# rensonnetg/microstructure_fingerprinting

Hardware: AMD Instinct MI355X
Metric: voxels/sec, 2-fascicle exhaustive NNLS, 782-atom x 200-measurement dictionary (higher is better)
Workload: dtype f64 (pairs ranked on split-f16 MFMA, short list re-evaluated in f64); 1 GPU; C2: 100000 voxels/GPU, 2 fascicles, 782 atoms x 200 measurements; voxels_per_gpu=100000, global_voxels=100000, atoms=782, measurements=200, ranks_in_group=1

## Files before the change

### microstructure_fingerprinting_amd/_lib.py

```python
import ctypes as C
import os

import numpy as np

_HERE = os.path.dirname(os.path.abspath(__file__))
LIB_PATH = os.path.join(_HERE, "libmfx.so")

MFX_OK, MFX_ERR_ARG, MFX_ERR_G_RANGE, MFX_ERR_NO_DEVICE, MFX_ERR_HIP, MFX_ERR_UNSUPPORTED, MFX_ERR_DIR_NORM = range(7)

_lib = None

EXPORTS = [
    "mfx_last_error", "mfx_device_count", "mfx_abi_version",
    "mfx_tables_create", "mfx_tables_destroy", "mfx_tables_num_atoms",
    "mfx_plan_create_multishell", "mfx_plan_create_explicit", "mfx_plan_destroy", "mfx_plan_status",
    "mfx_rotate", "mfx_rotate_dev", "mfx_rotate_cols", "mfx_rotate_cols_dev", "mfx_fit_batch", "mfx_fit_batch_rows", "mfx_fit_batch_volume", "mfx_volume_rows", "mfx_thread_release", "mfx_fit_batch_dev",
    "mfx_solve_exhaustive", "mfx_monte_carlo_average", "mfx_monte_carlo_average_dev", "mfx_cleanup_2fascicles", "mfx_cleanup_2fascicles_dev", "mfx_last_kernel_ms", "mfx_set_profiling", "mfx_debug_set_stamps", "mfx_debug_last_fallback_count", "mfx_debug_last_guard_count", "mfx_debug_last_counter", "mfx_debug_set_k2_screen", "mfx_debug_set_k2_wide", "mfx_debug_set_k2x_screen", "mfx_debug_set_k2_maxc", "mfx_debug_set_k2x_maxc", "mfx_debug_set_k2s_cap", "mfx_debug_set_k2s_images", "mfx_debug_set_k3_cap", "mfx_debug_set_force_generic", "mfx_debug_set_k3_screen",
]

MCF_EXPORTS = ["mfx_mcf_abi_version", "mfx_mcf_pgse", "mfx_mcf_dde"]

ROT2D_EXPORTS = ["mfx_rot2d_abi_version", "mfx_rot2d_create", "mfx_rot2d_destroy", "mfx_rot2d_rotate",
                 "mfx_rot2d_rotate_dev", "mfx_rot2d_rotate_cols", "mfx_rot2d_rotate_cols_dev"]

# ... 6 lines not shown
PREDICT_EXPORTS = ["mfx_predict_abi_version", "mfx_predict_dev", "mfx_predict", "mfx_sos_noise_dev", "mfx_sos_noise"]

PROFILE_EXPORTS = ["mfx_profile_abi_version", "mfx_profile_cut", "mfx_profile_max_atoms", "mfx_profile_dev", "mfx_profile",
                   "mfx_pair_objectives_dev", "mfx_pair_objectives"]

POST_EXPORTS = ["mfx_post_abi_version", "mfx_post_max_atoms", "mfx_post_dev", "mfx_post"]

WSOFT_EXPORTS = ["mfx_wsoft_abi_version", "mfx_wsoft_max_atoms", "mfx_wpost_dev", "mfx_wpost", "mfx_wprofile_dev", "mfx_wprofile",
                 "mfx_wpair_objectives_dev", "mfx_wpair_objectives"]

SOFT2D_EXPORTS = ["mfx_soft2d_abi_version", "mfx_soft2d_max_atoms", "mfx_post2d_dev", "mfx_post2d", "mfx_profile2d_dev",
                  "mfx_profile2d"]

W2D_EXPORTS = ["mfx_w2d_abi_version", "mfx_w2d_max_atoms", "mfx_wfit2d_batch_dev", "mfx_wfit2d_batch", "mfx_wpost2d_dev",
               "mfx_wpost2d", "mfx_wprofile2d_dev", "mfx_wprofile2d", "mfx_w2d_debug_set_force_explicit"]


class MfxError(RuntimeError):
    pass


def lib():
    global _lib
    if _lib is not None:
        return _lib
    if not os.path.exists(LIB_PATH):
        raise MfxError("HIP extension %s not found: run `python -c 'import __graft_entry__ as g; g.build()'` "
                       "(or `make -C microstructure_fingerprinting_amd/csrc`). There is no CPU fallback." % LIB_PATH)
    L = C.CDLL(LIB_PATH)
    dp = C.POINTER(C.c_double)
# ... 46 lines not shown
    L.mfx_debug_set_k2_wide.restype = None
    L.mfx_debug_set_k2x_screen.argtypes = [C.c_int]
    L.mfx_debug_set_k2x_screen.restype = None
    L.mfx_debug_set_k2_maxc.argtypes = [C.c_int]
    L.mfx_debug_set_k2_maxc.restype = None
    L.mfx_debug_set_k2s_cap.argtypes = [C.c_int]
    L.mfx_debug_set_k2s_cap.restype = None
    L.mfx_debug_set_k3_cap.argtypes = [C.c_int]
    L.mfx_debug_set_k3_cap.restype = None
    L.mfx_debug_set_force_generic.argtypes = [C.c_int]
    L.mfx_debug_set_force_generic.restype = None
    L.mfx_debug_set_k3_screen.argtypes = [C.c_int]
    L.mfx_debug_set_k3_screen.restype = None
    L.mfx_debug_set_k2s_images.argtypes = [C.c_int]
    L.mfx_debug_set_k2s_images.restype = None
    L.mfx_mcf_abi_version.restype = C.c_int
    for fn in ("mfx_mcf_pgse", "mfx_mcf_dde"):
        getattr(L, fn).argtypes = [dp, dp, C.c_int, dp, C.c_int64, dp, dp, C.c_int64, dp, C.c_double, dp]
        getattr(L, fn).restype = C.c_int
    L.mfx_rot2d_abi_version.restype = C.c_int
    L.mfx_rot2d_create.argtypes = [dp, C.c_int, ip, ip, C.c_int, ip, dp, ip, ip, ip, dp, C.c_int, ip, dp, dp, C.c_int,
                                   C.c_int, C.c_double, C.c_double, C.c_int, C.POINTER(vp)]
    L.mfx_rot2d_destroy.argtypes = [vp]
    L.mfx_rot2d_destroy.restype = None
    L.mfx_rot2d_rotate.argtypes = [vp, dp, C.c_int64, dp, ip]
    L.mfx_rot2d_rotate_dev.argtypes = [vp, vp, C.c_int64, vp, vp, vp]
    L.mfx_rot2d_rotate_cols.argtypes = [vp, dp, ip, C.c_int64, dp, ip]
    L.mfx_rot2d_rotate_cols_dev.argtypes = [vp, vp, vp, C.c_int64, vp, vp, vp]
    L.mfx_fit2d_abi_version.restype = C.c_int
    L.mfx_fit2d_max_atoms.argtypes = [vp, C.c_int]
# ... 88 lines not shown
```

### microstructure_fingerprinting_amd/csrc/fit_k2.hip

```cpp
#pragma once
#include <type_traits>

#include "mfx_device.h"
#include "nnls_small.h"

typedef double d4 __attribute__((ext_vector_type(4)));

#define MFX_WG 512
#define MFX_MAXC 256
#define MFX_S_CAP 2048
#define MFX_DET_REL 1e-8
#define MFX_A12_REL 4e-14

struct FitK2Args {
  TablesDev T;
  PlanDev P;
  const double* Y;
  const double* peaks;
  int peaks_ld;
  const int* vox_list;
  const int* list_count;
  double* params;
  int num_params;
  int maxfasc;
  int csf_on, ear_on;
  unsigned long long* stamps;
  int* fb_count;
  int* fb_list;
  int maxc;
  int scap;
  const double* xc;
  struct Cand* xl_cand;
  int* xl_cnt;
  double* xl_mrg;
  int xl_cap;
  int vox_base;
  int* audit;
};

#ifdef MFX_STAMPS
#define MFX_STAMP(i) do { if (a.stamps && tid == 0) a.stamps[(size_t)blockIdx.x * 16 + (i)] = __builtin_amdgcn_s_memtime(); } while (0)
#else
#define MFX_STAMP(i) do { } while (0)
#endif

struct Cand {
  double score;
  int i, j;
};

__device__ __forceinline__ double wave_max(double v) {
#pragma unroll
// ... 560 lines not shown
```

### microstructure_fingerprinting_amd/csrc/k2s_launch.h

```cpp
#pragma once
#include "mfx_host.h"
#include "fit_k2s.hip"

template <int KS, bool BR, int NB>
static int launch_k2s_t(const FitK2Args& a, int nvox, hipStream_t st) {
  MfxThread& T = mfx_thread();
  const size_t lds = mfx_k2s_lds_bytes(KS, a.T.N, BR, NB);
  auto kern = mfx_fit_k2s_kernel<KS, BR, NB>;
  HIPCHK(hipFuncSetAttribute((const void*)kern, hipFuncAttributeMaxDynamicSharedMemorySize, (int)lds));
  StreamMem fbm(st);
  HIPCHK(fbm.alloc(sizeof(int) * ((size_t)nvox + 8)));
  int* fb = fbm.as<int>();
  HIPCHK(hipMemsetAsync(fb, 0, 8 * sizeof(int), st));
  if (int rc = mfx_prof_begin(st)) return rc;
  FitK2Args aa = a;
  aa.stamps = T.stamps;
  aa.fb_count = fb;
  aa.fb_list = fb + 8;
  aa.audit = fb + 2;
  aa.scap = T.k2s_cap ? T.k2s_cap : MFX_S_CAP;
  hipLaunchKernelGGL(kern, dim3(nvox), dim3(512), lds, st, aa);
  HIPCHK(hipGetLastError());
  if (int rc = mfx_prof_end(st)) return rc;
  FitK2Args ab = a;
  ab.vox_list = fb + 8;
  ab.list_count = fb;
  if (int rc = mfx_launch_k2_f64(ab, nvox, st, false)) return rc;
  if (int rc = mfx_fb_accumulate(fb, 2, st)) return rc;
  return mfx_fb_accumulate_audit(fb + 2, st);
}

#define MFX_K2S_TU(KS_, NAME_)                                                            \
  int NAME_(const FitK2Args& a, int nvox, hipStream_t st, bool br, int NB) {              \
    if (NB == 3) return br ? launch_k2s_t<KS_, true, 3>(a, nvox, st) : launch_k2s_t<KS_, false, 3>(a, nvox, st); \
    return br ? launch_k2s_t<KS_, true, 2>(a, nvox, st) : launch_k2s_t<KS_, false, 2>(a, nvox, st);              \
// ... 2 lines not shown
```

### microstructure_fingerprinting_amd/csrc/k2s_shared.h

```cpp
#pragma once

template <int KS, int NB, bool BR, bool XC, int PQF>
struct K2sLds {
  static constexpr int MP = KS * 16;
  double* smem;
  _Float16* sBh;
  _Float16* sBl;
  double* s_y;
  double* s_t0;
  double* s_red;
  Cand* s_cand;
  unsigned long long* s_thr;
  int* s_r0;
  int* s_cnt;
  float* s_t0f;
  float* s_Zf;
  float* s_cs;
  float* s_yf;
  float* s_pq;
  double* s_t1;
  double* s_tG;
  double* s_dG;
  int* s_r1;
  int* s_rs;
// ... 7 lines not shown
    s_t0 = s_y + MP;
    s_red = s_t0 + 2 * MP;
    s_cand = (Cand*)(s_red + 32);
    s_thr = (unsigned long long*)(s_cand + MFX_S_CAP);
    s_r0 = (int*)(s_thr + 2);
    s_cnt = s_r0 + 2 * MP;
    s_t0f = (float*)(s_cnt + 4);
    s_Zf = s_t0f + 2 * MP;
    s_cs = s_Zf + 2 * NP;
    s_yf = s_cs + 2 * NP;
    s_pq = s_yf + MP;
    s_t1 = (double*)(s_pq + PQF);
    s_tG = s_t1 + (BR ? 2 * MP : 0);
    s_dG = s_tG + (BR ? MP : 0);
    s_r1 = (int*)(s_dG + (BR ? MP : 0));
    s_rs = BR ? s_r1 + 2 * MP : s_r0;
    s_evl4 = s_r1 + (BR ? 4 * MP : 0);
    s_xf = (float*)(s_evl4 + (KS < 8 ? MFX_S_CAP : 0));
    s_uf = s_xf + (XC ? MP : 0);
  }
};
#define K2S_UNPACK(L) \
  [[maybe_unused]] _Float16* const sBh = (L).sBh; \
  [[maybe_unused]] _Float16* const sBl = (L).sBl; \
  [[maybe_unused]] double* const s_y = (L).s_y; \
  [[maybe_unused]] double* const s_t0 = (L).s_t0; \
  [[maybe_unused]] double* const s_red = (L).s_red; \
  [[maybe_unused]] Cand* const s_cand = (L).s_cand; \
  [[maybe_unused]] unsigned long long* const s_thr = (L).s_thr; \
  [[maybe_unused]] int* const s_r0 = (L).s_r0; \
  [[maybe_unused]] int* const s_cnt = (L).s_cnt; \
  [[maybe_unused]] float* const s_t0f = (L).s_t0f; \
  [[maybe_unused]] float* const s_Zf = (L).s_Zf; \
  [[maybe_unused]] float* const s_cs = (L).s_cs; \
  [[maybe_unused]] float* const s_yf = (L).s_yf; \
  [[maybe_unused]] float* const s_pq = (L).s_pq; \
  [[maybe_unused]] double* const s_t1 = (L).s_t1; \
  [[maybe_unused]] double* const s_tG = (L).s_tG; \
  [[maybe_unused]] double* const s_dG = (L).s_dG; \
  [[maybe_unused]] int* const s_r1 = (L).s_r1; \
  [[maybe_unused]] int* const s_rs = (L).s_rs; \
  [[maybe_unused]] int* const s_evl4 = (L).s_evl4; \
  [[maybe_unused]] float* const s_xf = (L).s_xf; \
  [[maybe_unused]] float* const s_uf = (L).s_uf;

struct K2sVoxel {
  double y_sq;
  double yx;
  double ramp;
  double dc_eff;
  double mrg;
  double etol;
};

__device__ __forceinline__ unsigned k2s_audit_hash(int vox) {
  unsigned h = (unsigned)vox * 2654435761u;
  h ^= h >> 15; h *= 2246822519u; h ^= h >> 13; h *= 3266489917u; h ^= h >> 16;
  return h;
}
__device__ __forceinline__ int k2s_audit_key(unsigned h, int ntiles_reg, int ntiles) {
// ... 9 lines not shown
    atomicMax(&L.s_thr[1], mfx_nonneg_bits(fmin(old, 1e300)));
  }
  L.s_cand[idx].score = S;
  L.s_cand[idx].i = i;
  L.s_cand[idx].j = j;
}

template <int KS, int NB, bool BR, bool XC, int PQF, int WG>
__device__ __forceinline__ K2sVoxel k2s_prologue(const FitK2Args& a, const K2sLds<KS, NB, BR, XC, PQF>& L, const int vox, const int tid) {
  constexpr int MP = KS * 16, NW = WG / 64;
  const int lane = tid & 63, wave = tid >> 6;
  const int M = a.P.M, N = a.T.N, ldn = a.T.ldn;
  const int NP = (N + 31) & ~31;
  [[maybe_unused]] double* const smem = L.smem;
  K2S_UNPACK(L);

  MFX_STAMP(0);
  const double* __restrict__ yv = a.Y + (size_t)vox * M;
  const double* __restrict__ pk = a.peaks + (size_t)vox * a.peaks_ld;
  for (int m = tid; m < MP; m += WG) { const double v = (m < M) ? yv[m] : 0.0; s_y[m] = v; s_yf[m] = (float)v; }
  for (int idx = tid; idx < 2 * MP; idx += WG) {
    const int k = idx / MP, m = idx - k * MP;
    RowDesc rd;
    rd.r0 = a.T.P; rd.t0 = 0.0; rd.r1 = -1; rd.t1 = 0.0;
    if (m < M) rd = mfx_row_desc(a.T, a.P, m, pk[3 * k], pk[3 * k + 1], pk[3 * k + 2]);
    s_r0[idx] = rd.r0 * ldn;
    s_t0[idx] = rd.t0;
    if constexpr (!BR) {
      s_t0f[idx] = (float)rd.t0;
    } else {
      s_r1[idx] = rd.r1 < 0 ? -1 : rd.r1 * ldn;
      s_t1[idx] = rd.t1;
      if (k == 0) { s_tG[m] = (m < M) ? a.P.tG[m] : 0.0; s_dG[m] = (m < M) ? a.P.dG[m] : 1.0; }
      int rs = a.T.P;
      double ts = 0.0;
      if (m < M) {
        const int sg = a.P.s_scr[m], st = a.P.offs[2 * sg], cn = a.P.offs[2 * sg + 1];
        const double u = mfx_absdot(a.P.g + 3 * m, pk[3 * k], pk[3 * k + 1], pk[3 * k + 2]);
        int j = mfx_searchsorted_left(a.P.xs + st, cn, u);
        j = j < 1 ? 1 : (j > cn - 1 ? cn - 1 : j);
        rs = st + j - 1;
        ts = u - a.P.xs[rs];
      }
      s_rs[idx] = rs * ldn;
      s_t0f[idx] = (float)ts;
    }
  }
  if (tid == 0) { s_cnt[0] = 0; s_cnt[1] = 0; s_thr[0] = 0ull; s_thr[1] = 0ull; ((float*)(s_red + 30))[0] = __int_as_float(0x7fc00000); }
  if constexpr (XC) {
    for (int m = tid; m < MP; m += WG) s_xf[m] = (m < M) ? (float)a.xc[m] : 0.0f;
    if (tid < 2) ((unsigned long long*)s_red)[24 + tid] = 0ull;
  }
  if (tid < 2) mfx_check_dir(a.P, pk + 3 * tid, vox);
  __syncthreads();

  const float2* __restrict__ tab32 = a.P.tab32s;
  auto tab32x2_at = [&](int ro, int n) -> f32x4 { return *(const f32x4*)((const char*)tab32 + ((unsigned)(ro + n) << 3)); };

  MFX_STAMP(1);
  double y_sq_v = 0.0;
  for (int m = 0; m < M; ++m) y_sq_v += s_y[m] * s_y[m];
  const double y_sq = mfx_readlane_f64(y_sq_v, 0);
  double rsh_v = 1.0, yx_v = 0.0;
  if constexpr (XC) {
    double h = 0.0, xy = 0.0;
    for (int m = 0; m < M; ++m) { const double xv = (double)s_xf[m]; h = fma(xv, xv, h); xy = fma(xv, (double)s_yf[m], xy); }
    rsh_v = h > 0.0 ? 1.0 / sqrt(h) : 0.0;
    yx_v = xy * rsh_v;
  }
  const double rsh = mfx_readlane_f64(rsh_v, 0), yx = mfx_readlane_f64(yx_v, 0);
  const double y_sq_p = XC ? fmax(y_sq - yx * yx, 0.0) : y_sq;
  double my_s[2] = {0.0, 0.0};
  int my_n[2] = {0, 0};
  {
    const int VH = ((N + 1) / 2 + 63) & ~63;
    const int npass = (VH + WG - 1) / WG;
#pragma unroll 1
    for (int kd = XC ? 0 : 1; kd < 2; ++kd) {
    double ms_cur = 0.0, rm2_cur = 1.0;
    int mn_cur = 0;
    for (int p0 = 0; p0 < npass; p0 += 2) {
      int kq[2], nq[2];
      bool wact[2];
      double a2[2][2], ay[2][2], au[2][2];
#pragma unroll
      for (int q = 0; q < 2; ++q) {
        const int v = tid + WG * (p0 + q);
        kq[q] = kd;
        nq[q] = 2 * v;
        wact[q] = __any((p0 + q < npass) && (nq[q] < N));
        a2[q][0] = a2[q][1] = ay[q][0] = ay[q][1] = 0.0;
        au[q][0] = au[q][1] = 0.0;
      }
      int ncl[2];
#pragma unroll
      for (int q = 0; q < 2; ++q) ncl[q] = min(nq[q], ldn - 2);
      f32x4 dbuf[2][2][4];
      auto issue = [&](int m4, auto stc) {
        constexpr int st = decltype(stc)::value;
#pragma unroll
        for (int q = 0; q < 2; ++q) {
          if (wact[q]) {
            const i32x4 r = *(const i32x4*)(s_rs + kq[q] * MP + m4);
#pragma unroll
            for (int e = 0; e < 4; ++e) dbuf[st][q][e] = tab32x2_at(r[e], ncl[q]);
          }
        }
      };
      auto accumulate = [&](int m4, auto stc) {
        constexpr int st = decltype(stc)::value;
        const f32x4 yv = *(const f32x4*)(s_yf + m4);
        f32x4 xv = {0.0f, 0.0f, 0.0f, 0.0f};
        if constexpr (XC) xv = *(const f32x4*)(s_xf + m4);
#pragma unroll
        for (int q = 0; q < 2; ++q) {
          if (wact[q]) {
            const f32x4 t = *(const f32x4*)(s_t0f + kq[q] * MP + m4);
#pragma unroll
            for (int e = 0; e < 4; ++e) {
              const f32x4 d = dbuf[st][q][e];
              const double d0 = (double)fmaf(d[1], t[e], d[0]), d1 = (double)fmaf(d[3], t[e], d[2]);
              const double ye = (double)yv[e];
              a2[q][0] = fma(d0, d0, a2[q][0]);
              ay[q][0] = fma(ye, d0, ay[q][0]);
              a2[q][1] = fma(d1, d1, a2[q][1]);
              ay[q][1] = fma(ye, d1, ay[q][1]);
              if constexpr (XC) {
                const double xe = (double)xv[e];
                au[q][0] = fma(xe, d0, au[q][0]);
                au[q][1] = fma(xe, d1, au[q][1]);
              }
            }
          }
        }
      };
      issue(0, std::integral_constant<int, 0>{});
      for (int m4 = 0; m4 < MP; m4 += 8) {
        issue(m4 + 4, std::integral_constant<int, 1>{});
        accumulate(m4, std::integral_constant<int, 0>{});
        if (m4 + 8 < MP) issue(m4 + 8, std::integral_constant<int, 0>{});
        accumulate(m4 + 4, std::integral_constant<int, 1>{});
      }
#pragma unroll
      for (int q = 0; q < 2; ++q) {
#pragma unroll
        for (int u = 0; u < 2; ++u) {
          const int k = kq[q], n = nq[q] + u;
          if (p0 + q < npass && n < NP) {
            const bool act = n < N;
            if constexpr (!XC) {
              const double inv = (act && a2[q][u] > 0.0) ? 1.0 / sqrt(a2[q][u]) : 0.0;
              const double z = ay[q][u] * inv;
              s_Zf[k * NP + n] = act ? (float)z : -1e30f;
              s_cs[NP + n] = (act && inv > 0.0) ? (float)sqrt(a2[q][u]) : 0.0f;
              const double s = z > 0.0 ? z * z : 0.0;
              if (act && s > ms_cur) { ms_cur = s; mn_cur = n; }
// ... 469 lines not shown
```

### microstructure_fingerprinting_amd/csrc/k2w_launch.h

```cpp
#pragma once
#include "mfx_host.h"
#include "fit_k2w.hip"

template <int KS, int TL, bool BR, int NB>
static int launch_k2w_t(const FitK2Args& a, int nvox, hipStream_t st) {
  MfxThread& T = mfx_thread();
  const size_t lds = mfx_k2w_lds_bytes(KS, a.T.N, BR, NB, TL);
  if (lds > 160 * 1024) return mfx_fail(MFX_ERR_UNSUPPORTED, "wide K=2 kernel needs %zu B of LDS (> 160 KiB): N=%d too large", lds, a.T.N);
  auto kern = mfx_fit_k2w_kernel<KS, TL, BR, NB>;
  HIPCHK(hipFuncSetAttribute((const void*)kern, hipFuncAttributeMaxDynamicSharedMemorySize, (int)lds));
  StreamMem fbm(st);
  HIPCHK(fbm.alloc(sizeof(int) * ((size_t)nvox + 8)));
  int* fb = fbm.as<int>();
  HIPCHK(hipMemsetAsync(fb, 0, 8 * sizeof(int), st));
  if (int rc = mfx_prof_begin(st)) return rc;
  FitK2Args aa = a;
  aa.stamps = T.stamps;
  aa.fb_count = fb;
  aa.fb_list = fb + 8;
  aa.audit = fb + 2;
  aa.scap = T.k2s_cap ? T.k2s_cap : MFX_S_CAP;
  hipLaunchKernelGGL(kern, dim3(nvox), dim3(256), lds, st, aa);
  HIPCHK(hipGetLastError());
  if (int rc = mfx_prof_end(st)) return rc;
  FitK2Args ab = a;
  ab.vox_list = fb + 8;
  ab.list_count = fb;
  if (int rc = mfx_launch_k2_f64(ab, nvox, st, false)) return rc;
  if (int rc = mfx_fb_accumulate(fb, 2, st)) return rc;
  return mfx_fb_accumulate_audit(fb + 2, st);
}

#define MFX_K2W_TU(KS_, TL_, NB_, NAME_)                                                    \
  int NAME_(const FitK2Args& a, int nvox, hipStream_t st, bool br) {                        \
    return br ? launch_k2w_t<KS_, TL_, true, NB_>(a, nvox, st) : launch_k2w_t<KS_, TL_, false, NB_>(a, nvox, st); \
  }
// ... 1 lines not shown
```

### microstructure_fingerprinting_amd/csrc/mfx_api.hip

```cpp
#include "mfx_host.h"

#include <algorithm>
#include <chrono>
#include <cmath>
#include <cstdarg>
#include <cstdio>
#include <cstdlib>
#include <cstring>
#include <memory>
#include <string>
#include <vector>

#include "fit_small.hip"
#include "extras.hip"
#include "rotate.hip"
#include "solve_generic.hip"
#include "solve_k3.hip"
#include "fit_k3.hip"
#include "mc_average.hip"
#include "cleanup.hip"
#include "mfx_device.h"

MfxThread& mfx_thread() {
  static thread_local MfxThread t;
// ... 98 lines not shown
  HIPCHK(hipEventRecord(T.ev0, st));
  return MFX_OK;
}
int mfx_prof_end(hipStream_t st) {
  MfxThread& T = mfx_thread();
  if (!T.profiling) return MFX_OK;
  HIPCHK(hipEventRecord(T.ev1, st));
  T.ev_launches = 1;
  T.ev_valid = true;
  return MFX_OK;
}
__global__ void mfx_fb_add_kernel(const int* __restrict__ cnt, int n, int* __restrict__ tot) {
  if (threadIdx.x < n) atomicAdd(&tot[threadIdx.x], cnt[threadIdx.x]);
}
__global__ void mfx_fb_audit_kernel(const int* __restrict__ cnt, int* __restrict__ tot) {
  if (threadIdx.x == 0) { atomicAdd(&tot[0], cnt[0]); atomicMax(&tot[1], cnt[1]); atomicAdd(&tot[2], cnt[2]); }
}
static int fb_setup() {
  MfxThread& T = mfx_thread();
  int dev = 0;
  HIPCHK(hipGetDevice(&dev));
  if (T.fb_dev && T.fb_device == dev) return MFX_OK;
  if (T.fb_dev) { (void)hipFree(T.fb_dev); T.fb_dev = nullptr; }
  HIPCHK(hipMalloc((void**)&T.fb_dev, MFX_NCOUNTERS * sizeof(int)));
  T.fb_device = dev;
  if (!T.fb_host) {
    HIPCHK(hipHostMalloc((void**)&T.fb_host, MFX_NCOUNTERS * sizeof(int), hipHostMallocDefault));
    HIPCHK(hipEventCreateWithFlags(&T.fb_event, hipEventDisableTiming));
  }
  return MFX_OK;
}
// ... 49 lines not shown
  return (double)ms / T.ev_launches;
}
extern "C" int mfx_debug_last_fallback_count(void) { return fb_read(0); }
extern "C" int mfx_debug_last_guard_count(void) { return fb_read(1); }
extern "C" int mfx_debug_last_counter(int which) { return (which >= 0 && which < MFX_NCOUNTERS) ? fb_read(which) : -1; }
extern "C" void mfx_debug_set_k2_screen(int enabled) { mfx_thread().k2_screen = enabled ? 1 : 0; }
extern "C" void mfx_debug_set_k2_wide(int mode) { mfx_thread().k2_wide = mode == 1 ? 1 : (mode == 0 ? 0 : 2); }
extern "C" void mfx_debug_set_k2x_screen(int on) { mfx_thread().k2x_screen = on ? 1 : 0; }
extern "C" void mfx_debug_set_stamps(void* dev_ptr) { mfx_thread().stamps = (unsigned long long*)dev_ptr; }
extern "C" void mfx_debug_set_k2_maxc(int maxc) { mfx_thread().k2_maxc = (maxc < 0 || maxc > MFX_MAXC) ? MFX_MAXC : maxc; }
extern "C" void mfx_debug_set_k2x_maxc(int maxc) { mfx_thread().k2x_maxc = (maxc < 0 || maxc > MFX_XMAXC) ? MFX_XMAXC : maxc; }
extern "C" void mfx_debug_set_k3_cap(int cap) { mfx_thread().k3_cap = cap > 0 ? cap : 0; }
extern "C" void mfx_debug_set_force_generic(int enabled) { mfx_thread().force_generic = enabled ? 1 : 0; }
extern "C" void mfx_debug_set_k3_screen(int enabled) { mfx_thread().k3_screen = enabled ? 1 : 0; }
extern "C" void mfx_debug_set_k2s_images(int nb) { mfx_thread().k2s_nb = (nb == 2) ? 2 : 0; }
extern "C" void mfx_debug_set_k2s_cap(int cap) {
  int c = 4;
  while (2 * c <= cap) c *= 2;
  mfx_thread().k2s_cap = (cap <= 0 || c >= MFX_S_CAP) ? 0 : c;
}

struct mfx_tables {
  int device = 0;
  TablesDev d{};
  std::vector<double> h_x, h_G, h_Y;
  double scr_scale = 1.0;
  std::vector<int> h_off;
  void* dx = nullptr;
  void* doff = nullptr;
  void* dtab = nullptr;
// ... 117 lines not shown
  HIPCHK(hipMemcpy(p->dg, g.data(), sizeof(double) * 3 * M, hipMemcpyHostToDevice));
  HIPCHK(hipMemcpy(p->dslo, slo.data(), sizeof(int) * M, hipMemcpyHostToDevice));
  HIPCHK(hipMemcpy(p->dshi, shi.data(), sizeof(int) * M, hipMemcpyHostToDevice));
  HIPCHK(hipMemcpy(p->dtG, tG.data(), sizeof(double) * M, hipMemcpyHostToDevice));
  HIPCHK(hipMemcpy(p->ddG, dG.data(), sizeof(double) * M, hipMemcpyHostToDevice));
  p->d.M = M;
  p->d.g = (const double*)p->dg;
  p->d.s_lo = (const int*)p->dslo;
  p->d.s_hi = (const int*)p->dshi;
  p->d.tG = (const double*)p->dtG;
  p->d.dG = (const double*)p->ddG;
  p->d.any_bracket = 0;
  p->d.normalise = normalise;
  for (int m = 0; m < M; ++m) p->d.any_bracket |= (shi[m] >= 0);
  p->d.tab32s = t->d.tab32; p->d.xs = nullptr; p->d.offs = nullptr; p->d.s_scr = nullptr;
  if (p->d.any_bracket) {
    const int S = t->d.S, N = t->d.N, ldn = t->d.ldn, P = t->d.P;
    const double* X = t->h_x.data();
    const double* Y = t->h_Y.data();
    const int* off = t->h_off.data();
    auto interp = [&](int s, double u, int n) {
      const int o = off[s], Ps = off[s + 1] - o;
      int j = (int)(std::lower_bound(X + o, X + o + Ps, u) - (X + o));
      j = j < 1 ? 1 : (j > Ps - 1 ? Ps - 1 : j);
      const int r = o + j - 1;
      const double sl = (Y[(size_t)(r + 1) * N + n] - Y[(size_t)r * N + n]) / (X[r + 1] - X[r]);
      return sl * (u - X[r]) + Y[(size_t)r * N + n];
    };
    struct VS { int lo, hi; double w; };
    std::vector<VS> vs;
// ... 41 lines not shown
        offs.push_back((int)base);
        offs.push_back(K);
      }
      sscr[m] = t->d.S + v;
    }
    HIPCHK(hipMalloc(&p->dtab32s, sizeof(float2) * tabs.size()));
    HIPCHK(hipMalloc(&p->dxs, sizeof(double) * xs.size()));
    HIPCHK(hipMalloc(&p->doffs, sizeof(int) * offs.size()));
    HIPCHK(hipMalloc(&p->dsscr, sizeof(int) * M));
    HIPCHK(hipMemcpy(p->dtab32s, tabs.data(), sizeof(float2) * tabs.size(), hipMemcpyHostToDevice));
    HIPCHK(hipMemcpy(p->dxs, xs.data(), sizeof(double) * xs.size(), hipMemcpyHostToDevice));
    HIPCHK(hipMemcpy(p->doffs, offs.data(), sizeof(int) * offs.size(), hipMemcpyHostToDevice));
    HIPCHK(hipMemcpy(p->dsscr, sscr.data(), sizeof(int) * M, hipMemcpyHostToDevice));
    p->d.tab32s = (const float2*)p->dtab32s; p->d.xs = (const double*)p->dxs;
    p->d.offs = (const int*)p->doffs; p->d.s_scr = (const int*)p->dsscr;
  }
  *out = p.release();
  return MFX_OK;
}

extern "C" int mfx_plan_create_multishell(const mfx_tables* t, const double* scheme, int M, mfx_plan** out) {
  if (!t || !scheme || !out || M < 1) return fail(MFX_ERR_ARG, "mfx_plan_create_multishell: bad argument");
  const int S = t->d.S;
  std::vector<double> g(3 * (size_t)M), tG(M, 0.0), dG(M, 1.0);
  std::vector<int> slo(M, 0), shi(M, -1);
  for (int m = 0; m < M; ++m) {
    const double* r = scheme + 7 * (size_t)m;
    g[3 * m] = r[0]; g[3 * m + 1] = r[1]; g[3 * m + 2] = r[2];
    const double G = r[3];
    int sx = -1;
// ... 37 lines not shown
  if (!p) return fail(MFX_ERR_ARG, "mfx_plan_status: null plan");
  if (int rc = require_device(p->t->device)) return rc;
  int st[4] = {0, 0, 0, 0};
  HIPCHK(hipMemcpyAsync(st, p->dstatus, sizeof(st), hipMemcpyDeviceToHost, (hipStream_t)stream));
  HIPCHK(hipStreamSynchronize((hipStream_t)stream));
  if (st[0] == 0) return MFX_OK;
  HIPCHK(hipMemsetAsync(p->dstatus, 0, sizeof(st), (hipStream_t)stream));
  if (st[0] & MFX_ST_DIR_NORM)
    return fail(MFX_ERR_DIR_NORM, "Orientation vector of the new signal must have unit norm (voxel %d of the batch).", st[1]);
  return fail(MFX_ERR_HIP, "fit kernels reported status 0x%x", st[0]);
}

size_t mfx_k2s_lds_bytes(int KS, int N, bool bracket, int NB) {
  const size_t MP = (size_t)KS * 16, NP = ((size_t)N + 31) / 32 * 32;
  return (size_t)2 * NB * KS * 512 * 2 + 8 * (MP + 2 * MP + 32) + sizeof(Cand) * MFX_S_CAP + 16 + 4 * (2 * MP + 4) + 4 * (2 * MP) + 4 * (4 * NP) + 4 * MP + 4 * 8 * 64 +
         (bracket ? 48 * MP : 0) + (KS < 8 ? 4 * MFX_S_CAP : 0);
}

size_t mfx_k2sx_lds_bytes(int KS, int N, bool bracket, int NB) {
  const size_t MP = (size_t)KS * 16, NP = ((size_t)N + 31) / 32 * 32;
  return mfx_k2s_lds_bytes(KS, N, bracket, NB) + 4 * MP + 8 * NP;
}

size_t mfx_k2w_lds_bytes(int KS, int N, bool bracket, int NB, int TL) {
  const size_t MP = (size_t)KS * 16, NP = ((size_t)N + 31) / 32 * 32;
  return (size_t)2 * NB * KS * 512 * 2 + 8 * (MP + 2 * MP + 32) + sizeof(Cand) * MFX_S_CAP + 16 + 4 * (2 * MP + 4) + 4 * (2 * MP) + 4 * (4 * NP) + 4 * MP +
         4 * 4 * TL * 64 + (bracket ? 48 * MP : 0) + (KS < 8 ? 4 * MFX_S_CAP : 0);
}

size_t mfx_k2wx_lds_bytes(int KS, int N, bool bracket, int NB, int TL) {
  const size_t MP = (size_t)KS * 16, NP = ((size_t)N + 31) / 32 * 32;
  return mfx_k2w_lds_bytes(KS, N, bracket, NB, TL) + 4 * MP + 8 * NP;
}

static int launch_k2(const FitK2Args& a, int nvox, hipStream_t st) {
  MfxThread& T = mfx_thread();
  if (T.k2_screen < 0) { const char* e = getenv("MFX_K2_SCREEN"); T.k2_screen = (e && e[0] == '0') ? 0 : 1; }
  if (T.k2_wide < 0) { const char* e = getenv("MFX_K2_WIDE"); T.k2_wide = e ? (e[0] == '1' ? 1 : (e[0] == '0' ? 0 : 2)) : 2; }
  const int M = a.P.M;
  const bool br = a.P.any_bracket != 0;
  if (T.k2_screen && mfx_k2_f64_fits(a)) {
    const bool wide_ok = T.k2_wide != 0;
// ... 1097 lines not shown
```

### microstructure_fingerprinting_amd/csrc/mfx_device.h

```cpp
#pragma once
#include <hip/hip_runtime.h>
#include <stdint.h>

struct TablesDev {
  int S, N, ldn, P;
  const double* x;
  const int* off;
  const double2* tab;
  const float2* tab32;
  const double* G_un;
};

struct PlanDev {
  int M;
  const double* g;
  const int* s_lo;
  const int* s_hi;
  const double* tG;
  const double* dG;
  int any_bracket;
  int normalise;
  const float2* tab32s;
  const double* xs;
  const int* offs;
  const int* s_scr;
  int* status;
};

#define MFX_ST_DIR_NORM 1

__device__ __forceinline__ void mfx_check_dir(const PlanDev& P, const double* __restrict__ pk, int vox) {
  if (P.normalise) return;
  const double nrm = sqrt((pk[0] * pk[0] + pk[1] * pk[1]) + pk[2] * pk[2]);
  if (!(fabs(1.0 - nrm) <= 1e-3) && P.status) {
    atomicOr(P.status, MFX_ST_DIR_NORM);
    P.status[1] = vox;
  }
}

struct RowDesc {
// ... 57 lines not shown
```

### microstructure_fingerprinting_amd/csrc/mfx_host.h

```cpp
#pragma once
#include "../../include/mfx.h"

#include <hip/hip_runtime.h>

#include <string>
#include <vector>

#include "fit_k2.hip"
#include "fit_k2x.hip"

#define MFX_NCOUNTERS 12

struct MfxThread {
  std::string err;
  hipEvent_t ev0 = nullptr, ev1 = nullptr;
  int ev_launches = 0;
  bool ev_valid = false;
  bool profiling = false;
  unsigned long long* stamps = nullptr;
  int k2_pipe = -1;
  int k2_maxc = MFX_MAXC;
  int k2x_maxc = MFX_XMAXC;
  int k2s_nb = 0;
  int k2s_cap = 0;
  int force_generic = 0;
  int k3_screen = 1;
  int k3_cap = 0;
  int k3_batch = -1;
  int k2_screen = -1;
  int k2x_screen = -1;
  int k2_wide = -1;
  int* fb_dev = nullptr;
  int* fb_host = nullptr;
  int fb_device = -1;
  hipEvent_t fb_event = nullptr;
  bool fb_pending = false;
  void* stage[2] = {nullptr, nullptr};
  size_t stage_bytes = 0;
  hipStream_t s_copy = nullptr, s_comp = nullptr;
// ... 6 lines not shown
    hipStream_t stream = nullptr;
    std::vector<void*> blocks;
    std::vector<size_t> sizes;
    size_t cur = 0, off = 0;
    int live = 0;
    unsigned long long used = 0;
  };
  std::vector<Arena> arenas;
  unsigned long long arena_clock = 0;
  hipStream_t s_lane[4] = {nullptr, nullptr, nullptr, nullptr};
  hipEvent_t ev_lane[5] = {nullptr, nullptr, nullptr, nullptr, nullptr};
  int lane_device = -1;
};

MfxThread& mfx_thread();
int mfx_fail(int code, const char* fmt, ...) __attribute__((format(printf, 2, 3)));

#define HIPCHK(x)                                                                                   \
  do {                                                                                              \
    hipError_t e_ = (x);                                                                            \
    if (e_ != hipSuccess) return mfx_fail(MFX_ERR_HIP, "%s failed: %s", #x, hipGetErrorString(e_)); \
  } while (0)

struct DevMem {
  void* p = nullptr;
  DevMem() = default;
  DevMem(const DevMem&) = delete;
  DevMem& operator=(const DevMem&) = delete;
  ~DevMem() { if (p) (void)hipFree(p); }
  hipError_t alloc(size_t bytes) { return hipMalloc(&p, bytes ? bytes : 8); }
// ... 49 lines not shown
```

### microstructure_fingerprinting_amd/csrc/tu_k2x.hip

```cpp
#include "mfx_host.h"

#include <algorithm>
#include <cstdlib>

#define MFX_XLCAP 256

static size_t k2x_lds_bytes(int ksteps, bool bracket, int NP, int nw, int nbuf, int ntup, int M, int NX) {
  const size_t MP = (size_t)ksteps * 4;
  size_t dbl = (size_t)nbuf * MP * 16 + MP + 2 * MP + (bracket ? 2 * MP + 2 * MP : 0) + 4 * (size_t)NP + (size_t)nw * 16 * MFX_XS +
               2 * 16 * MFX_XS + MFX_XS + MFX_XS * MFX_XS + 24 + MFX_XS +
               (4 * MFX_XS + 2) + (size_t)nw * 16 + 2 * 16 + 2;
  dbl += (size_t)M * NX;
  return dbl * 8 + sizeof(CandX) * MFX_XMAXC + sizeof(FamX) * MFX_XFAM + sizeof(ProjC) * ((size_t)nw * 16 + 2 * 16) * ntup +
         sizeof(int) * (2 * MP + (bracket ? 2 * MP : 0) + 4 + 2 * nw) + sizeof(QItem) * (size_t)nw * MFX_XQ;
}

static int k2x_lds_plan(FitK2XArgs& a, int ksteps, bool bracket, int nw, int nbuf, int ntup, size_t* lds) {
  const size_t cap = 160 * 1024;
  a.xx_in_lds = 1;
  *lds = k2x_lds_bytes(ksteps, bracket, a.T.ldn, nw, nbuf, ntup, a.P.M, a.X.NX);
  if (*lds <= cap) return MFX_OK;
  a.xx_in_lds = 0;
  *lds = k2x_lds_bytes(ksteps, bracket, a.T.ldn, nw, nbuf, ntup, 0, 0);
  if (*lds <= cap) return MFX_OK;
// ... 59 lines not shown
  HIPCHK(hipMemsetAsync(cnt.p, 0, 4 * sizeof(int), st));
  HIPCHK(hipMemsetAsync(fbm.p, 0, 4 * sizeof(int), st));
  int* fb = fbm.as<int>();
  a.ws = ws.as<double>();
  a.maxc = T.k2x_maxc;
  a.stamps = T.stamps;
  a.ovf_count = cnt.as<int>();
  a.xl_cand = xlc.as<Cand>(); a.xl_cnt = xln.as<int>(); a.xl_mrg = xlm.as<double>(); a.xl_cap = cap;
  a.fb_count = fb; a.fb_list = fb + 4; a.list_count = nullptr;
  FitK2Args s{};
  s.T = a.T; s.P = a.P; s.Y = a.Y; s.peaks = a.peaks; s.peaks_ld = a.peaks_ld; s.vox_list = a.vox_list; s.list_count = nullptr;
  s.params = a.params; s.num_params = a.num_params; s.maxfasc = a.maxfasc; s.csf_on = a.csf_on; s.ear_on = a.ear_on;
  s.stamps = nullptr; s.fb_count = fb; s.fb_list = fb + 4; s.maxc = 0; s.scap = T.k2s_cap ? T.k2s_cap : MFX_S_CAP;
  s.xc = a.X.x; s.xl_cand = xlc.as<Cand>(); s.xl_cnt = xln.as<int>(); s.xl_mrg = xlm.as<double>(); s.xl_cap = cap;
  s.audit = aud.as<int>();
  if (int rc = mfx_prof_begin(st)) return rc;
  for (int base = 0; base < nvox; base += big) {
    const int n = std::min(big, nvox - base);
    s.vox_base = base;
    const int M = a.P.M;
    if (int rc = (M < 128 ? mfx_launch_k2sx_ks8 : (M <= 200 ? mfx_launch_k2sx_ks13 : (M < 384 ? mfx_launch_k2wx_ks24 : mfx_launch_k2wx_ks35)))(s, n, st, BRACKET)) return rc;
    a.vox_base = base;
    hipLaunchKernelGGL(kern_list, dim3(n), dim3(NW * 64), lds, st, a);
  }
  FitK2XArgs b = a;
  b.vox_list = fb + 4; b.list_count = fb; b.xl_cand = nullptr; b.xl_cnt = nullptr;
  for (int base = 0; base < nvox; base += chunk) {
    b.vox_base = base;
    hipLaunchKernelGGL(kern_full, dim3(std::min(chunk, nvox - base)), dim3(NW * 64), lds, st, b);
  }
// ... 32 lines not shown
```

Baseline: 1.108 million voxels/s.

## Sort screening rows by table row and collapse shared-row runs into moment sums

Before the pair-screening pass, measurements are sorted by their table row offset for the second fascicle. Rows that share a table row are merged into precomputed moment sums (count, t, t², y, yt, x, xt), so the screening loop does one table fetch per distinct row instead of one per measurement. Singleton rows keep the old per-row path through compacted buffers. This adds a per-voxel O(M²) rank sort, extra LDS scratch, several barriers and double-precision accumulation, and it slightly changes rounding in the screening scores.

```diff
diff --git a/include/mfx_k2s.h b/include/mfx_k2s.h
--- /dev/null
+++ b/include/mfx_k2s.h
@@ -0,0 +1,12 @@
+#ifndef MFX_K2S_H
+#define MFX_K2S_H
+#ifdef __cplusplus
+extern "C" {
+#endif
+
+void mfx_debug_set_k2s_rowsort(int on);
+
+#ifdef __cplusplus
+}
+#endif
+#endif
diff --git a/microstructure_fingerprinting_amd/_lib.py b/microstructure_fingerprinting_amd/_lib.py
--- a/microstructure_fingerprinting_amd/_lib.py
+++ b/microstructure_fingerprinting_amd/_lib.py
@@ -44,6 +44,8 @@
 
 W2D_EXPORTS = ["mfx_w2d_abi_version", "mfx_w2d_max_atoms", "mfx_wfit2d_batch_dev", "mfx_wfit2d_batch", "mfx_wpost2d_dev",
                "mfx_wpost2d", "mfx_wprofile2d_dev", "mfx_wprofile2d", "mfx_w2d_debug_set_force_explicit"]
+
+K2S_EXPORTS = ["mfx_debug_set_k2s_rowsort"]
 
 
 class MfxError(RuntimeError):
@@ -120,6 +122,8 @@
     L.mfx_debug_set_k3_screen.restype = None
     L.mfx_debug_set_k2s_images.argtypes = [C.c_int]
     L.mfx_debug_set_k2s_images.restype = None
+    L.mfx_debug_set_k2s_rowsort.argtypes = [C.c_int]
+    L.mfx_debug_set_k2s_rowsort.restype = None
     L.mfx_mcf_abi_version.restype = C.c_int
     for fn in ("mfx_mcf_pgse", "mfx_mcf_dde"):
         getattr(L, fn).argtypes = [dp, dp, C.c_int, dp, C.c_int64, dp, dp, C.c_int64, dp, C.c_double, dp]
diff --git a/microstructure_fingerprinting_amd/csrc/fit_k2.hip b/microstructure_fingerprinting_amd/csrc/fit_k2.hip
--- a/microstructure_fingerprinting_amd/csrc/fit_k2.hip
+++ b/microstructure_fingerprinting_amd/csrc/fit_k2.hip
@@ -36,6 +36,7 @@
   int xl_cap;
   int vox_base;
   int* audit;
+  int rowsort;
 };
 
 #ifdef MFX_STAMPS
diff --git a/microstructure_fingerprinting_amd/csrc/k2s_launch.h b/microstructure_fingerprinting_amd/csrc/k2s_launch.h
--- a/microstructure_fingerprinting_amd/csrc/k2s_launch.h
+++ b/microstructure_fingerprinting_amd/csrc/k2s_launch.h
@@ -19,6 +19,7 @@
   aa.fb_list = fb + 8;
   aa.audit = fb + 2;
   aa.scap = T.k2s_cap ? T.k2s_cap : MFX_S_CAP;
+  aa.rowsort = mfx_k2s_rowsort_on(a);
   hipLaunchKernelGGL(kern, dim3(nvox), dim3(512), lds, st, aa);
   HIPCHK(hipGetLastError());
   if (int rc = mfx_prof_end(st)) return rc;
diff --git a/microstructure_fingerprinting_amd/csrc/k2s_shared.h b/microstructure_fingerprinting_amd/csrc/k2s_shared.h
--- a/microstructure_fingerprinting_amd/csrc/k2s_shared.h
+++ b/microstructure_fingerprinting_amd/csrc/k2s_shared.h
@@ -45,8 +45,8 @@
     s_tG = s_t1 + (BR ? 2 * MP : 0);
     s_dG = s_tG + (BR ? MP : 0);
     s_r1 = (int*)(s_dG + (BR ? MP : 0));
-    s_rs = BR ? s_r1 + 2 * MP : s_r0;
-    s_evl4 = s_r1 + (BR ? 4 * MP : 0);
+    s_rs = s_r1 + (BR ? 2 * MP : 0);
+    s_evl4 = s_rs + 2 * MP;
     s_xf = (float*)(s_evl4 + (KS < 8 ? MFX_S_CAP : 0));
     s_uf = s_xf + (XC ? MP : 0);
   }
@@ -75,6 +75,29 @@
   [[maybe_unused]] float* const s_xf = (L).s_xf; \
   [[maybe_unused]] float* const s_uf = (L).s_uf;
 
+template <int MP>
+struct K2sRuns {
+  int* key;
+  int* pc;
+  int* sg_ro;
+  float* sg_t;
+  float* sg_y;
+  float* sg_x;
+  int* mr_ro;
+  double* mr_sum;
+  static constexpr int BYTES = 4 * (6 * MP + 32) + 64 * (MP / 2 + 8);
+  __device__ __forceinline__ K2sRuns(double* smem) {
+    key = (int*)smem;
+    pc = key + MP;
+    sg_ro = pc + 32;
+    sg_t = (float*)(sg_ro + MP);
+    sg_y = sg_t + MP;
+    sg_x = sg_y + MP;
+    mr_ro = (int*)(sg_x + MP);
+    mr_sum = (double*)(mr_ro + MP);
+  }
+};
+
 struct K2sVoxel {
   double y_sq;
   double yx;
@@ -114,6 +137,8 @@
   const int NP = (N + 31) & ~31;
   [[maybe_unused]] double* const smem = L.smem;
   K2S_UNPACK(L);
+  static_assert(K2sRuns<MP>::BYTES <= NB * KS * 2048, "the scratch of the screening order must fit the chunk images");
+  const K2sRuns<MP> R(smem);
 
   MFX_STAMP(0);
   const double* __restrict__ yv = a.Y + (size_t)vox * M;
@@ -128,6 +153,8 @@
     s_t0[idx] = rd.t0;
     if constexpr (!BR) {
       s_t0f[idx] = (float)rd.t0;
+      s_rs[idx] = rd.r0 * ldn;
+      if (k == 1) R.key[m] = (m < M) ? (rd.r0 << 10) | m : 0x7fffffff;
     } else {
       s_r1[idx] = rd.r1 < 0 ? -1 : rd.r1 * ldn;
       s_t1[idx] = rd.t1;
@@ -144,6 +171,7 @@
       }
       s_rs[idx] = rs * ldn;
       s_t0f[idx] = (float)ts;
+      if (k == 1) R.key[m] = (m < M) ? (rs << 10) | m : 0x7fffffff;
     }
   }
   if (tid == 0) { s_cnt[0] = 0; s_cnt[1] = 0; s_thr[0] = 0ull; s_thr[1] = 0ull; ((float*)(s_red + 30))[0] = __int_as_float(0x7fc00000); }
@@ -153,6 +181,108 @@
   }
   if (tid < 2) mfx_check_dir(a.P, pk + 3 * tid, vox);
   __syncthreads();
+
+  int ns8 = 0, nm8 = 0;
+  if (a.rowsort) {
+    constexpr int NIT = (MP + WG - 1) / WG;
+    int pos[NIT], q0[NIT], q1[NIT];
+    float qa[NIT], qb[NIT], qy[NIT], qx[NIT];
+#pragma unroll
+    for (int it = 0; it < NIT; ++it) {
+      const int m = tid + it * WG;
+      pos[it] = 0; q0[it] = 0; q1[it] = 0; qa[it] = 0.0f; qb[it] = 0.0f; qy[it] = 0.0f; qx[it] = 0.0f;
+      if (m < M) {
+        const int key = R.key[m];
+        int c = 0;
+        for (int j = 0; j < M; j += 4) {
+          const i32x4 k4 = *(const i32x4*)(R.key + j);
+#pragma unroll
+          for (int e = 0; e < 4; ++e) c += (k4[e] < key) ? 1 : 0;
+        }
+        pos[it] = c;
+        q0[it] = s_rs[m]; q1[it] = s_rs[MP + m];
+        qa[it] = s_t0f[m]; qb[it] = s_t0f[MP + m];
+        qy[it] = s_yf[m];
+        if constexpr (XC) qx[it] = s_xf[m];
+      }
+    }
+    __syncthreads();
+#pragma unroll
+    for (int it = 0; it < NIT; ++it) {
+      const int m = tid + it * WG, p = pos[it];
+      if (m < M) {
+        s_rs[p] = q0[it]; s_rs[MP + p] = q1[it];
+        s_t0f[p] = qa[it]; s_t0f[MP + p] = qb[it];
+        s_yf[p] = qy[it];
+        if constexpr (XC) s_xf[p] = qx[it];
+      }
+    }
+    __syncthreads();
+    int kind[NIT], ix_s[NIT], ix_m[NIT];
+    const unsigned long long below = (1ull << lane) - 1ull;
+#pragma unroll
+    for (int it = 0; it < NIT; ++it) {
+      const int p = tid + it * WG;
+      bool sg = false, mh = false;
+      if (p < M) {
+        const int ro = s_rs[MP + p];
+        const bool head = p == 0 || s_rs[MP + p - 1] != ro;
+        const bool last = p + 1 >= M || s_rs[MP + p + 1] != ro;
+        sg = head && last;
+        mh = head && !last;
+      }
+      const unsigned long long bs = __ballot(sg), bm = __ballot(mh);
+      if (lane == 0) R.pc[it * NW + wave] = __popcll(bs) | (__popcll(bm) << 16);
+      kind[it] = sg ? 1 : (mh ? 2 : 0);
+      ix_s[it] = __popcll(bs & below);
+      ix_m[it] = __popcll(bm & below);
+    }
+    __syncthreads();
+    int tot_s = 0, tot_m = 0;
+    for (int w = 0; w < NIT * NW; ++w) {
+      const int v = R.pc[w];
+#pragma unroll
+      for (int it = 0; it < NIT; ++it)
+        if (w == it * NW + wave) { ix_s[it] += tot_s; ix_m[it] += tot_m; }
+      tot_s += v & 0xffff;
+      tot_m += v >> 16;
+    }
+    tot_s = __builtin_amdgcn_readfirstlane(tot_s);
+    tot_m = __builtin_amdgcn_readfirstlane(tot_m);
+#pragma unroll
+    for (int it = 0; it < NIT; ++it) {
+      const int p = tid + it * WG;
+      if (kind[it] == 1) {
+        const int i = ix_s[it];
+        R.sg_ro[i] = s_rs[MP + p];
+        R.sg_t[i] = s_t0f[MP + p];
+        R.sg_y[i] = s_yf[p];
+        if constexpr (XC) R.sg_x[i] = s_xf[p];
+      } else if (kind[it] == 2) {
+        const int i = ix_m[it], ro = s_rs[MP + p];
+        double cnt = 0.0, St = 0.0, Stt = 0.0, Sy = 0.0, Syt = 0.0, Sx = 0.0, Sxt = 0.0;
+        for (int r = p; r < M && s_rs[MP + r] == ro; ++r) {
+          const double t = (double)s_t0f[MP + r], y = (double)s_yf[r];
+          cnt += 1.0; St += t; Stt = fma(t, t, Stt); Sy += y; Syt = fma(y, t, Syt);
+          if constexpr (XC) { const double x = (double)s_xf[r]; Sx += x; Sxt = fma(x, t, Sxt); }
+        }
+        R.mr_ro[i] = ro;
+        double* o = R.mr_sum + 8 * i;
+        o[0] = cnt; o[1] = 2.0 * St; o[2] = Stt; o[3] = Sy; o[4] = Syt; o[5] = Sx; o[6] = Sxt; o[7] = 0.0;
+      }
+    }
+    ns8 = (tot_s + 7) & ~7;
+    nm8 = (tot_m + 7) & ~7;
+    if (tid < 8) {
+      if (tot_s + tid < ns8) { R.sg_ro[tot_s + tid] = a.T.P * ldn; R.sg_t[tot_s + tid] = 0.0f; R.sg_y[tot_s + tid] = 0.0f; R.sg_x[tot_s + tid] = 0.0f; }
+      if (tot_m + tid < nm8) {
+        R.mr_ro[tot_m + tid] = a.T.P * ldn;
+        for (int e = 0; e < 8; ++e) R.mr_sum[8 * (tot_m + tid) + e] = 0.0;
+      }
+    }
+    if (tid == 0 && a.audit) atomicAdd(a.audit + 3, tot_s + tot_m);
+    __syncthreads();
+  }
 
   const float2* __restrict__ tab32 = a.P.tab32s;
   auto tab32x2_at = [&](int ro, int n) -> f32x4 { return *(const f32x4*)((const char*)tab32 + ((unsigned)(ro + n) << 3)); };
@@ -179,6 +309,12 @@
     for (int kd = XC ? 0 : 1; kd < 2; ++kd) {
     double ms_cur = 0.0, rm2_cur = 1.0;
     int mn_cur = 0;
+    const bool runs = a.rowsort && kd == 1;
+    const int* const rsb = runs ? R.sg_ro : s_rs + kd * MP;
+    const float* const tfb = runs ? R.sg_t : s_t0f + kd * MP;
+    const float* const yfb = runs ? R.sg_y : s_yf;
+    [[maybe_unused]] const float* const xfb = runs ? R.sg_x : s_xf;
+    const int nrow = runs ? ns8 : MP;
     for (int p0 = 0; p0 < npass; p0 += 2) {
       int kq[2], nq[2];
       bool wact[2];
@@ -196,12 +332,12 @@
 #pragma unroll
       for (int q = 0; q < 2; ++q) ncl[q] = min(nq[q], ldn - 2);
       f32x4 dbuf[2][2][4];
-      auto issue = [&](int m4, auto stc) {
+      auto issue = [&](const int* rb, int m4, auto stc) {
         constexpr int st = decltype(stc)::value;
 #pragma unroll
         for (int q = 0; q < 2; ++q) {
           if (wact[q]) {
-            const i32x4 r = *(const i32x4*)(s_rs + kq[q] * MP + m4);
+            const i32x4 r = *(const i32x4*)(rb + m4);
 #pragma unroll
             for (int e = 0; e < 4; ++e) dbuf[st][q][e] = tab32x2_at(r[e], ncl[q]);
           }
@@ -209,13 +345,13 @@
       };
       auto accumulate = [&](int m4, auto stc) {
         constexpr int st = decltype(stc)::value;
-        const f32x4 yv = *(const f32x4*)(s_yf + m4);
+        const f32x4 yv = *(const f32x4*)(yfb + m4);
         f32x4 xv = {0.0f, 0.0f, 0.0f, 0.0f};
-        if constexpr (XC) xv = *(const f32x4*)(s_xf + m4);
+        if constexpr (XC) xv = *(const f32x4*)(xfb + m4);
 #pragma unroll
         for (int q = 0; q < 2; ++q) {
           if (wact[q]) {
-            const f32x4 t = *(const f32x4*)(s_t0f + kq[q] * MP + m4);
+            const f32x4 t = *(const f32x4*)(tfb + m4);
 #pragma unroll
             for (int e = 0; e < 4; ++e) {
               const f32x4 d = dbuf[st][q][e];
@@ -234,12 +370,51 @@
           }
         }
       };
-      issue(0, std::integral_constant<int, 0>{});
-      for (int m4 = 0; m4 < MP; m4 += 8) {
-        issue(m4 + 4, std::integral_constant<int, 1>{});
+      auto accumulate_runs = [&](int g4, auto stc) {
+        constexpr int st = decltype(stc)::value;
+#pragma unroll
+        for (int e = 0; e < 4; ++e) {
+          const double* sm = R.mr_sum + 8 * (g4 + e);
+          const double2 c0 = *(const double2*)sm, c1 = *(const double2*)(sm + 2), c2 = *(const double2*)(sm + 4);
+          double sxt = 0.0;
+          if constexpr (XC) sxt = sm[6];
+#pragma unroll
+          for (int q = 0; q < 2; ++q) {
+            if (wact[q]) {
+              const f32x4 d = dbuf[st][q][e];
+#pragma unroll
+              for (int u = 0; u < 2; ++u) {
+                const double yl = (double)d[2 * u], sl = (double)d[2 * u + 1];
+                a2[q][u] = fma(yl, fma(c0.x, yl, c0.y * sl), a2[q][u]);
+                a2[q][u] = fma(c1.x * sl, sl, a2[q][u]);
+                ay[q][u] = fma(c1.y, yl, ay[q][u]);
+                ay[q][u] = fma(c2.x, sl, ay[q][u]);
+                if constexpr (XC) {
+                  au[q][u] = fma(c2.y, yl, au[q][u]);
+                  au[q][u] = fma(sxt, sl, au[q][u]);
+                }
+              }
+            }
+          }
+        }
+      };
+      if (nrow > 0) issue(rsb, 0, std::integral_constant<int, 0>{});
+      for (int m4 = 0; m4 < nrow; m4 += 8) {
+        issue(rsb, m4 + 4, std::integral_constant<int, 1>{});
         accumulate(m4, std::integral_constant<int, 0>{});
-        if (m4 + 8 < MP) issue(m4 + 8, std::integral_constant<int, 0>{});
+        if (m4 + 8 < nrow) issue(rsb, m4 + 8, std::integral_constant<int, 0>{});
         accumulate(m4 + 4, std::integral_constant<int, 1>{});
+      }
+      if (runs) {
+        if (nm8 > 0) issue(R.mr_ro, 0, std::integral_constant<int, 0>{});
+        for (int g4 = 0; g4 < nm8; g4 += 8) {
+          issue(R.mr_ro, g4 + 4, std::integral_constant<int, 1>{});
+          accumulate_runs(g4, std::integral_constant<int, 0>{});
+          if (g4 + 8 < nm8) issue(R.mr_ro, g4 + 8, std::integral_constant<int, 0>{});
+          accumulate_runs(g4 + 4, std::integral_constant<int, 1>{});
+        }
+#pragma unroll
+        for (int q = 0; q < 2; ++q) { a2[q][0] = fmax(a2[q][0], 0.0); a2[q][1] = fmax(a2[q][1], 0.0); }
       }
 #pragma unroll
       for (int q = 0; q < 2; ++q) {
diff --git a/microstructure_fingerprinting_amd/csrc/k2w_launch.h b/microstructure_fingerprinting_amd/csrc/k2w_launch.h
--- a/microstructure_fingerprinting_amd/csrc/k2w_launch.h
+++ b/microstructure_fingerprinting_amd/csrc/k2w_launch.h
@@ -20,6 +20,7 @@
   aa.fb_list = fb + 8;
   aa.audit = fb + 2;
   aa.scap = T.k2s_cap ? T.k2s_cap : MFX_S_CAP;
+  aa.rowsort = mfx_k2s_rowsort_on(a);
   hipLaunchKernelGGL(kern, dim3(nvox), dim3(256), lds, st, aa);
   HIPCHK(hipGetLastError());
   if (int rc = mfx_prof_end(st)) return rc;
diff --git a/microstructure_fingerprinting_amd/csrc/mfx_api.hip b/microstructure_fingerprinting_amd/csrc/mfx_api.hip
--- a/microstructure_fingerprinting_amd/csrc/mfx_api.hip
+++ b/microstructure_fingerprinting_amd/csrc/mfx_api.hip
@@ -136,7 +136,7 @@
   if (threadIdx.x < n) atomicAdd(&tot[threadIdx.x], cnt[threadIdx.x]);
 }
 __global__ void mfx_fb_audit_kernel(const int* __restrict__ cnt, int* __restrict__ tot) {
-  if (threadIdx.x == 0) { atomicAdd(&tot[0], cnt[0]); atomicMax(&tot[1], cnt[1]); atomicAdd(&tot[2], cnt[2]); }
+  if (threadIdx.x == 0) { atomicAdd(&tot[0], cnt[0]); atomicMax(&tot[1], cnt[1]); atomicAdd(&tot[2], cnt[2]); atomicAdd(&tot[3], cnt[3]); }
 }
 static int fb_setup() {
   MfxThread& T = mfx_thread();
@@ -216,6 +216,7 @@
 extern "C" void mfx_debug_set_force_generic(int enabled) { mfx_thread().force_generic = enabled ? 1 : 0; }
 extern "C" void mfx_debug_set_k3_screen(int enabled) { mfx_thread().k3_screen = enabled ? 1 : 0; }
 extern "C" void mfx_debug_set_k2s_images(int nb) { mfx_thread().k2s_nb = (nb == 2) ? 2 : 0; }
+extern "C" void mfx_debug_set_k2s_rowsort(int on) { mfx_thread().k2s_rowsort = on ? 1 : 0; }
 extern "C" void mfx_debug_set_k2s_cap(int cap) {
   int c = 4;
   while (2 * c <= cap) c *= 2;
@@ -363,6 +364,7 @@
   p->d.normalise = normalise;
   for (int m = 0; m < M; ++m) p->d.any_bracket |= (shi[m] >= 0);
   p->d.tab32s = t->d.tab32; p->d.xs = nullptr; p->d.offs = nullptr; p->d.s_scr = nullptr;
+  p->d.rows_scr = t->d.P + 1;
   if (p->d.any_bracket) {
     const int S = t->d.S, N = t->d.N, ldn = t->d.ldn, P = t->d.P;
     const double* X = t->h_x.data();
@@ -434,6 +436,7 @@
     HIPCHK(hipMemcpy(p->dsscr, sscr.data(), sizeof(int) * M, hipMemcpyHostToDevice));
     p->d.tab32s = (const float2*)p->dtab32s; p->d.xs = (const double*)p->dxs;
     p->d.offs = (const int*)p->doffs; p->d.s_scr = (const int*)p->dsscr;
+    p->d.rows_scr = (int)(tabs.size() / (size_t)ldn);
   }
   *out = p.release();
   return MFX_OK;
@@ -501,7 +504,7 @@
 size_t mfx_k2s_lds_bytes(int KS, int N, bool bracket, int NB) {
   const size_t MP = (size_t)KS * 16, NP = ((size_t)N + 31) / 32 * 32;
   return (size_t)2 * NB * KS * 512 * 2 + 8 * (MP + 2 * MP + 32) + sizeof(Cand) * MFX_S_CAP + 16 + 4 * (2 * MP + 4) + 4 * (2 * MP) + 4 * (4 * NP) + 4 * MP + 4 * 8 * 64 +
-         (bracket ? 48 * MP : 0) + (KS < 8 ? 4 * MFX_S_CAP : 0);
+         (bracket ? 48 * MP : 8 * MP) + (KS < 8 ? 4 * MFX_S_CAP : 0);
 }
 
 size_t mfx_k2sx_lds_bytes(int KS, int N, bool bracket, int NB) {
@@ -512,7 +515,7 @@
 size_t mfx_k2w_lds_bytes(int KS, int N, bool bracket, int NB, int TL) {
   const size_t MP = (size_t)KS * 16, NP = ((size_t)N + 31) / 32 * 32;
   return (size_t)2 * NB * KS * 512 * 2 + 8 * (MP + 2 * MP + 32) + sizeof(Cand) * MFX_S_CAP + 16 + 4 * (2 * MP + 4) + 4 * (2 * MP) + 4 * (4 * NP) + 4 * MP +
-         4 * 4 * TL * 64 + (bracket ? 48 * MP : 0) + (KS < 8 ? 4 * MFX_S_CAP : 0);
+         4 * 4 * TL * 64 + (bracket ? 48 * MP : 8 * MP) + (KS < 8 ? 4 * MFX_S_CAP : 0);
 }
 
 size_t mfx_k2wx_lds_bytes(int KS, int N, bool bracket, int NB, int TL) {
diff --git a/microstructure_fingerprinting_amd/csrc/mfx_device.h b/microstructure_fingerprinting_amd/csrc/mfx_device.h
--- a/microstructure_fingerprinting_amd/csrc/mfx_device.h
+++ b/microstructure_fingerprinting_amd/csrc/mfx_device.h
@@ -24,6 +24,7 @@
   const double* xs;
   const int* offs;
   const int* s_scr;
+  int rows_scr;
   int* status;
 };
 
diff --git a/microstructure_fingerprinting_amd/csrc/mfx_host.h b/microstructure_fingerprinting_amd/csrc/mfx_host.h
--- a/microstructure_fingerprinting_amd/csrc/mfx_host.h
+++ b/microstructure_fingerprinting_amd/csrc/mfx_host.h
@@ -1,5 +1,6 @@
 #pragma once
 #include "../../include/mfx.h"
+#include "../../include/mfx_k2s.h"
 
 #include <hip/hip_runtime.h>
 
@@ -23,6 +24,7 @@
   int k2x_maxc = MFX_XMAXC;
   int k2s_nb = 0;
   int k2s_cap = 0;
+  int k2s_rowsort = 1;
   int force_generic = 0;
   int k3_screen = 1;
   int k3_cap = 0;
@@ -59,6 +61,7 @@
 };
 
 MfxThread& mfx_thread();
+inline int mfx_k2s_rowsort_on(const FitK2Args& a) { return (mfx_thread().k2s_rowsort && a.P.rows_scr < (1 << 21) && a.P.M <= 1024) ? 1 : 0; }
 int mfx_fail(int code, const char* fmt, ...) __attribute__((format(printf, 2, 3)));
 
 #define HIPCHK(x)                                                                                   \
diff --git a/microstructure_fingerprinting_amd/csrc/tu_k2x.hip b/microstructure_fingerprinting_amd/csrc/tu_k2x.hip
--- a/microstructure_fingerprinting_amd/csrc/tu_k2x.hip
+++ b/microstructure_fingerprinting_amd/csrc/tu_k2x.hip
@@ -97,6 +97,7 @@
   s.stamps = nullptr; s.fb_count = fb; s.fb_list = fb + 4; s.maxc = 0; s.scap = T.k2s_cap ? T.k2s_cap : MFX_S_CAP;
   s.xc = a.X.x; s.xl_cand = xlc.as<Cand>(); s.xl_cnt = xln.as<int>(); s.xl_mrg = xlm.as<double>(); s.xl_cap = cap;
   s.audit = aud.as<int>();
+  s.rowsort = mfx_k2s_rowsort_on(s);
   if (int rc = mfx_prof_begin(st)) return rc;
   for (int base = 0; base < nvox; base += big) {
     const int n = std::min(big, nvox - base);
```

After: 1.114 million voxels/s (median of 6 runs). About the same (+0.5%).
